# miroslavradojevic/pnr

Hardware: AMD Instinct MI355X
Metric: Mvox/s traced (Frangi+SMC step) on 1024^3 synthetic stack; % HBM roofline (higher is better)
Workload: dtype f32 (+f64 3x3 eigen-solver)

## Files before the change

### pnr_amd/csrc/devbuf.h

```cpp
#pragma once
#include <hip/hip_runtime.h>
#include <algorithm>
#include <atomic>
#include <cstdint>

namespace pnr {

inline std::atomic<int64_t> live_device_bytes{0}, live_pinned_bytes{0};

template <typename T, bool Pinned>
class Buf {
    T *p_ = nullptr;
    size_t n_ = 0;
    static std::atomic<int64_t> &live() { return Pinned ? live_pinned_bytes : live_device_bytes; }

public:
    Buf() = default;
    Buf(const Buf &) = delete;
    Buf &operator=(const Buf &) = delete;
    Buf(Buf &&o) noexcept { adopt(o.p_, o.n_), o.release(); }
    Buf &operator=(Buf &&o) noexcept
    {
        if (this != &o) adopt(o.p_, o.n_), o.release();
        return *this;
    }
    ~Buf() { reset(); }

    T *get() const { return p_; }
    explicit operator bool() const { return p_ != nullptr; }
    size_t count() const { return n_; }

    hipError_t alloc(size_t count)
    {
        reset();
        const size_t n = std::max<size_t>(count, 1);
        void *q = nullptr;
        const hipError_t e = Pinned ? hipHostMalloc(&q, n * sizeof(T), hipHostMallocDefault) : hipMalloc(&q, n * sizeof(T));
        if (e == hipSuccess) adopt((T *)q, n);
        return e;
    }
    hipError_t reserve(size_t count) { return p_ && n_ >= count ? hipSuccess : alloc(count); }
    void reset()
    {
        if (T *p = release()) (void)(Pinned ? hipHostFree(p) : hipFree(p));
    }
    void adopt(T *p, size_t count)
    {
        reset();
        p_ = p, n_ = p ? count : 0;
        live() += (int64_t)(n_ * sizeof(T));
    }
    T *release()
    {
        T *p = p_;
        live() -= (int64_t)(n_ * sizeof(T));
        p_ = nullptr, n_ = 0;
        return p;
    }
};

// ... 5 lines not shown
```

### pnr_amd/csrc/smc_phased.hip

```cpp
#include "ctx.h"
#include "replay.h"
#include "stream_sched.h"
#ifdef PNR_EXPERIMENT_HOOKS
#include "../../scripts/probes/experiments/ph_sample_hooks.h"
#else
#define PNR_HOOK_AFTER_FULL_ITEM(seg_lane, cnt)
#endif
#include "smc_device.h"
#include <algorithm>
#include <cstdlib>

namespace {

enum { FL_RES = 0, FL_STOP = 1, FL_T = 2, FL_IT = 3, FL_DONE = 4, FL_OX = 5, FL_OY = 6, FL_OZ = 7, FL_Y0 = 8, FL_Y1 = 9, FL_Z0 = 10, FL_Z1 = 11, FL_FAST = 12, FL_NCH = 13, FL_PAUSE = 14, FL_N = 16 };
constexpr int PH_THREADS = 1024;
constexpr int PH_CS = 54;
constexpr int PH_PITCH = 56;
constexpr int PH_PLANE = PH_CS * PH_PITCH;
static_assert((size_t)PH_CS * PH_PLANE <= 160 * 1024, "the cube must fit the LDS of a CU");

struct PhState {
    float *part;
    float *prior;
    int *idxres;
    float *corr;
    float *xcs;
    int *flags;
    float *stash;
    long long trace_floats;
    int stash_base;
    unsigned char *cubes;
    int *list;
    int *cnt;
    int *ctr;
    int *uidx;
    int *cmap;
    int cap;
    int np_pad;
    int W;
    int dedup;
};

__device__ __forceinline__ unsigned int pose_hash(float x, float y, float z, float vx, float vy, float vz)
{
    unsigned int h = 0x811c9dc5u;
    const unsigned int w[6] = {__float_as_uint(x), __float_as_uint(y), __float_as_uint(z), __float_as_uint(vx), __float_as_uint(vy), __float_as_uint(vz)};
#pragma unroll
    for (int i = 0; i < 6; i++) {
        h = (h ^ w[i]) * 0x9e3779b1u;
        h ^= h >> 15;
    }
    h *= 0x85ebca6bu;
    h ^= h >> 13;
    return h;
}

__device__ __forceinline__ int last_group_stride(int rem) { return rem > 32 ? 64 : (rem > 16 ? 32 : 16); }


struct CubeRows { int ox, oy, oz, y0, y1, z0, z1; };
template <class DST>
__device__ __forceinline__ void stage_cube_rows(const Vol &V, const CubeRows &R, int wv, int nwv, int lane, DST *cube32)
{
    static_assert(PH_PITCH % 4 == 0 && PH_PITCH >= PH_CS && PH_PITCH <= 64, "one dword per lane, 16 lanes per row");
// ... 535 lines not shown
        const unsigned long long sst2 = __builtin_amdgcn_s_memtime();
        atomicAdd(&g_ph_stamps[5], sst1 - sst0);
        atomicAdd(&g_ph_stamps[6], sst2 - sst1);
        atomicAdd(&g_ph_stamps[7], 1ull);
    }
#endif
}

__device__ __forceinline__ float lds_seq_sum(const float *a, int n)
{
    float s = 0.f;
    int k = 0;
    for (; k + 8 <= n; k += 8) {
        float t[8];
#pragma unroll
        for (int j = 0; j < 8; j++) t[j] = a[k + j];
#pragma unroll
        for (int j = 0; j < 8; j++) s += t[j];
    }
    for (; k < n; k++) s += a[k];
    return s;
}

__global__ __launch_bounds__(256) void ph_update(Vol V, Tab T, PhState P, int np, int np_pad, int ni, int it_arg, int lp, float Kc, float znccth,
                                                  float neff_ratio, const unsigned char *__restrict__ den, int nodepervol, TraceOut O)
{
    extern __shared__ float lds[];
    const int tid = threadIdx.x, B = blockDim.x, S = T.nsig;
    PU_STAMP(ut0);
    if ((int)blockIdx.x >= P.cnt[lp]) return;
    const int tr = P.list[lp * P.cap + blockIdx.x];
    int *fl = P.flags + (i64)tr * FL_N;
    if (fl[FL_PAUSE]) return;
    const int it = it_arg >= 0 ? it_arg : fl[FL_IT];
    float *cur = lds;
    float *prvw = cur + np * PSTRIDE;
    float *prior = prvw + np;
    float *lhood = prior + np;
    float *csw = lhood + np;
    float *corr_ks = csw + np;
    float *sneff = corr_ks + S * np_pad;
    int *sres = (int *)(sneff + 2);
    float *sxc = (float *)(sres + 2);
    const bool tail = (it == ni) || (fl[FL_STOP] != 0);
    const int pending = it - 1;
    const int resampled_prev = fl[FL_RES];
    float *gpart = P.part + (i64)tr * 2 * np * PSTRIDE;
    float *gcur = gpart + (it & 1) * np * PSTRIDE;
    const float *gprv = gpart + ((it & 1) ^ 1) * np * PSTRIDE;
    float *xc_cur = P.xcs + (i64)tr * 16 + (it & 1) * 8;
    const float *xc_pen = P.xcs + (i64)tr * 16 + ((it & 1) ^ 1) * 8;
    int *gidx = P.idxres + (i64)tr * np;
    for (int e = tid; e < S * np_pad; e += B) corr_ks[e] = P.corr[(i64)tr * S * np_pad + e];
    const int cen = fl[FL_NCH] - 1;
    const int *cmap = P.cmap + (i64)tr * P.np_pad;
    if (!tail) {
// ... 2 lines not shown
    }
    __syncthreads();
    PU_STAMP(ut1);

    if (pending >= 0 && tid == 0) {
        float best = -FLT_MAX, bs = xc_pen[6];
        for (int s = 0; s < S; s++) {
            const float cv = corr_ks[s * np_pad + cen];
            if (cv > best) { best = cv; bs = T.sig[s]; }
        }
        float *xo = O.xc + ((i64)tr * ni + pending) * 8;
        xo[0] = xc_pen[0]; xo[1] = xc_pen[1]; xo[2] = xc_pen[2]; xo[3] = xc_pen[3]; xo[4] = xc_pen[4]; xo[5] = xc_pen[5];
        xo[6] = bs; xo[7] = best;
        if ((fl[FL_STOP] == 0 || fl[FL_STOP] == 3) && best < znccth) { fl[FL_STOP] = 2; fl[FL_T] = pending; }
    }
    if (tid == 0) sres[1] = fl[FL_STOP];
    __syncthreads();
    if (tail || sres[1] != 0) {
        if (tid == 0) {
            O.T[tr] = fl[FL_T];
            O.stop[tr] = fl[FL_STOP];
            fl[FL_DONE] = 1;
        }
        return;
    }

    PU_STAMP(ut2);
    for (int k = tid; k < np; k += B) {
        float best = -FLT_MAX, bs = 0.f;
        const int ck = cmap[k];
        for (int s = 0; s < S; s++) {
            const float cv = corr_ks[s * np_pad + ck];
            if (cv > best) { best = cv; bs = T.sig[s]; }
        }
        cur[k * PSTRIDE + PCORR] = best;
        cur[k * PSTRIDE + PSIG] = bs;
        lhood[k] = expf_libm(Kc * best);
    }
    __syncthreads();

    PU_STAMP(ut3);
    const bool carry = (it > 0) && !resampled_prev;
    const int lane = tid & 63, wv = tid >> 6;
    {
        const float wnorm_prior = lds_seq_sum(prior, np);
        for (int k = tid; k < np; k += B) {
            const double base = carry ? (double)prvw[k] : (1.0 / np);
// ... 95 lines not shown
                if (ui > csw[mid]) lo = mid + 1; else hi = mid;
            }
            gidx[k] = lo;
            if (it < O.dbg_iters && O.idxres) O.idxres[((i64)tr * O.dbg_iters + it) * np + k] = lo;
        }
    }
    if (tid == 0) {
        P.list[(lp ^ 1) * P.cap + atomicAdd(&P.cnt[lp ^ 1], 1)] = tr;
        fl[FL_IT] = it + 1;
    }
    for (int e = tid; e < np * PSTRIDE; e += B) gcur[e] = cur[e];
    if (it < O.dbg_iters && O.xfilt) {
        float *dst = O.xfilt + ((i64)tr * O.dbg_iters + it) * np * PSTRIDE;
        for (int e = tid; e < np * PSTRIDE; e += B) dst[e] = cur[e];
    }
#ifdef PNR_SMC_STAMPS
    if (tid == 0) {
        const unsigned long long ut7 = __builtin_amdgcn_s_memtime();
        atomicAdd(&g_pu_stamps[8], ut1 - ut0); atomicAdd(&g_pu_stamps[9], ut2 - ut1); atomicAdd(&g_pu_stamps[10], ut3 - ut2);
        atomicAdd(&g_pu_stamps[11], ut4 - ut3); atomicAdd(&g_pu_stamps[12], ut5 - ut4); atomicAdd(&g_pu_stamps[13], ut6 - ut5);
        atomicAdd(&g_pu_stamps[14], ut7 - ut6); atomicAdd(&g_pu_stamps[15], 1ull);
    }
#endif
}

__global__ __launch_bounds__(256) void ph_snapshot(const int4 *__restrict__ src, int4 *__restrict__ dst, int n4)
{
    const int i = blockIdx.x * 256 + threadIdx.x;
    if (i < n4) dst[i] = src[i];
}

__global__ __launch_bounds__(256) void ph_poll(PhState P, float *__restrict__ s6, int do_ctl, const int *__restrict__ pause, int np_,
                                                const int *__restrict__ resume, int nr, const int *__restrict__ new_slots,
                                                const float *__restrict__ new_s6, int m, int lp, int ni, unsigned char *__restrict__ den,
                                                const i64 *__restrict__ didx, const unsigned char *__restrict__ dval, int nt)
{
    if (blockIdx.x > 0) {
        const int i = ((int)blockIdx.x - 1) * (int)blockDim.x + (int)threadIdx.x;
        if (i < nt) den_raise(den, didx[i], dval[i]);
        return;
    }
    __shared__ int kept, cntv;
    if (threadIdx.x == 0) { cntv = P.cnt[lp]; kept = 0; }
    __syncthreads();
    int *list = P.list + (size_t)lp * P.cap, *tmp = P.list + (size_t)(lp ^ 1) * P.cap;
    if (do_ctl) {
        const int n = cntv;
        for (int j = threadIdx.x; j < np_; j += blockDim.x) P.flags[(i64)pause[j] * FL_N + FL_PAUSE] = 1;
        __syncthreads();
        if (np_ > 0) {
            for (int j = threadIdx.x; j < n; j += blockDim.x) {
                const int tr = list[j];
                if (!P.flags[(i64)tr * FL_N + FL_PAUSE]) tmp[atomicAdd(&kept, 1)] = tr;
            }
            __syncthreads();
            for (int j = threadIdx.x; j < kept; j += blockDim.x) list[j] = tmp[j];
            __syncthreads();
        } else if (threadIdx.x == 0) {
            kept = n;
        }
        __syncthreads();
        const int base = kept;
        for (int j = threadIdx.x; j < nr; j += blockDim.x) {
            P.flags[(i64)resume[j] * FL_N + FL_PAUSE] = 0;
            list[base + j] = resume[j];
        }
        __syncthreads();
        if (threadIdx.x == 0) cntv = base + nr;
        __syncthreads();
    }
    if (m > 0) {
        const int base = cntv;
        for (int j = threadIdx.x; j < m; j += blockDim.x) {
            const int slot = new_slots[j];
            for (int a = 0; a < 6; a++) s6[(i64)slot * 6 + a] = new_s6[(i64)j * 6 + a];
            int *fl = P.flags + (i64)slot * FL_N;
            for (int a = 0; a < FL_N; a++) fl[a] = 0;
            fl[FL_T] = ni;
            for (int a = 0; a < 16; a++) P.xcs[(i64)slot * 16 + a] = 0.f;
            list[base + j] = slot;
        }
        __syncthreads();
        if (threadIdx.x == 0) cntv = base + m;
        __syncthreads();
    }
    if (threadIdx.x == 0) P.cnt[lp] = cntv;
}

}

struct pnr_phased {
    static constexpr int RING = 8, MAXG = 4;
    int64_t cap_traces = 0, cap_dbg = 0;
    int64_t cap_stash = 0;
    int np = 0, np_pad = 0, S = 0, ni = 0;
    long long trace_floats = 0;
    PhState P{};
    struct {
        pnr::DevBuf<float> part, prior, corr, xcs, stash;
        pnr::DevBuf<int> idxres, list, cnt, ctr, uidx, cmap;
        pnr::DevBuf<unsigned char> cubes;
    } state;
    pnr::DevBuf<float> d_s6;
    TraceOut O{};
    TraceOutBufs out;
    pnr::PinBuf<int> h_cnt;
    hipEvent_t ev[RING] = {};
    pnr::PinBuf<pnr_xest> h_xc; pnr::PinBuf<int> h_flags, h_new; pnr::PinBuf<float> h_new_s6;
    pnr::PinBuf<int> h_ctl;
    pnr::PinBuf<long long> h_den_idx[MAXG];
    pnr::PinBuf<unsigned char> h_den_val[MAXG];
    int64_t stream_cap = 0;
    int stream_ni = 0;
    hipStream_t stg[MAXG] = {};
    hipEvent_t ev_start = nullptr;
    hipEvent_t ev_state[MAXG] = {};
    hipEvent_t ev_ctl[MAXG] = {};
};

static void phased_free(pnr_phased *h)
{
    h->state = {};
    h->d_s6.reset();
    h->out.reset();
    h->P = PhState{};
    h->O = TraceOut{};
    h->cap_traces = h->cap_dbg = 0;
    h->cap_stash = 0;
}

#ifdef PNR_SMC_STAMPS
extern "C" int pnr_debug_pu_fine(unsigned long long *out4, int reset)
{
    if (out4 && hipMemcpyFromSymbol(out4, HIP_SYMBOL(g_pu_fine), 64) != hipSuccess) return -1;
    if (reset) { unsigned long long z[8] = {}; if (hipMemcpyToSymbol(HIP_SYMBOL(g_pu_fine), z, 64) != hipSuccess) return -1; }
    return 0;
}

extern "C" int pnr_debug_pu_stamps(unsigned long long *out16, int reset)
{
    if (out16 && hipMemcpyFromSymbol(out16, HIP_SYMBOL(g_pu_stamps), 128) != hipSuccess) return -1;
    if (reset) { unsigned long long z[16] = {}; if (hipMemcpyToSymbol(HIP_SYMBOL(g_pu_stamps), z, 128) != hipSuccess) return -1; }
    return 0;
}

extern "C" int pnr_debug_ph_stamps(unsigned long long *out8, int reset)
{
    if (out8 && hipMemcpyFromSymbol(out8, HIP_SYMBOL(g_ph_stamps), 64) != hipSuccess) return -1;
    if (reset) { unsigned long long z[8] = {}; if (hipMemcpyToSymbol(HIP_SYMBOL(g_ph_stamps), z, 64) != hipSuccess) return -1; }
    return 0;
}
#endif

void pnr_phased_destroy(pnr_phased *h)
{
    if (!h) return;
    for (int r = 0; r < pnr_phased::RING; r++)
        if (h->ev[r]) (void)hipEventDestroy(h->ev[r]);
    for (int g = 1; g < pnr_phased::MAXG; g++)
        if (h->stg[g]) (void)hipStreamDestroy(h->stg[g]);
    if (h->ev_start) (void)hipEventDestroy(h->ev_start);
    for (hipEvent_t &e : h->ev_state) if (e) (void)hipEventDestroy(e);
    for (hipEvent_t &e : h->ev_ctl) if (e) (void)hipEventDestroy(e);
    delete h;
}

static bool sums_deep(const pnr_ctx *c, int active, int ngroups)
{
    if (c->opt.sums_deep >= 0) return c->opt.sums_deep != 0;
    return ngroups <= 1 || active <= c->opt.sums_deep_max;
}

static int share_scales(const pnr_ctx *c, int active)
{
    return (c->opt.share_scales && c->tab.guest_mask != 0 && active >= c->opt.share_min) ? 1 : 0;
}

static int ph_tbl(int np)
{
    int t = 64;
    while (t < 2 * np) t <<= 1;
    return t;
}

static size_t ph_predict_lds(int np, int dedup) { return dedup ? (size_t)(np * 8 + 2 * ph_tbl(np)) * 4 : (size_t)np * 8; }

// ... 17 lines not shown
{
    const dim3 grid((unsigned)(active * nsplit)), blk(PH_THREADS);
    if (P.cubes) {
        if (V.l == 1) hipLaunchKernelGGL((ph_sample<PH_CS, true, true>), grid, blk, cube_bytes, st, V, T, X, P, np, ni, it, lp, active, share);
        else hipLaunchKernelGGL((ph_sample<PH_CS, false, true>), grid, blk, cube_bytes, st, V, T, X, P, np, ni, it, lp, active, share);
    } else {
        if (V.l == 1) hipLaunchKernelGGL((ph_sample<PH_CS, true, false>), grid, blk, cube_bytes, st, V, T, X, P, np, ni, it, lp, active, share);
        else hipLaunchKernelGGL((ph_sample<PH_CS, false, false>), grid, blk, cube_bytes, st, V, T, X, P, np, ni, it, lp, active, share);
    }
}

struct PhEnv {
    Vol V; Tab T; TabX X; PhState P;
    int np, ni, S, np_pad, ng, ncu, max_split, dbg_iters;
    size_t cube_bytes, upd_lds;
    long long trace_floats;
    int64_t NT;
    pnr_phased *h;
};

struct StepTimers { bool on, chain_first, chain_rest; int weight; };

static void smc_step(pnr_ctx *c, const PhEnv &E, hipStream_t st, const PhState &P, int active, int it, int lp, int x10, int sharing,
                     const unsigned char *den, const TraceOut &O, const StepTimers &tm)
{
    const int np = E.np, ni = E.ni;
    const int nsplit = pick_nsplit(active, E.ncu, E.max_split, x10), share = share_scales(c, active);
    bool chain = tm.chain_first;
    auto tic = [&] { if (tm.on) c->tic(st, chain); chain = tm.chain_rest; };
    auto toc = [&](const char *group) { if (tm.on) c->toc(group, 1, st, tm.weight); };
    tic();
    hipLaunchKernelGGL(ph_predict, dim3(active), dim3(256), ph_predict_lds(np, P.dedup), st, E.T, E.X, P, (const float *)E.h->d_s6.get(), E.V, np, ni, it, lp, PH_CS, ph_tbl(np));
    toc("smc_predict");
    if (P.cubes) {
        tic();
        hipLaunchKernelGGL(ph_cube, dim3((unsigned)(active * PH_CUBE_SPLIT)), dim3(PH_CUBE_THREADS), 0, st, E.V, P, lp, active);
        toc("smc_cube");
    }
    tic();
    launch_sample(st, E.V, E.T, E.X, P, np, ni, it, lp, active, nsplit, E.cube_bytes, share);
    toc("smc");
    tic();
    launch_sums(st, E.T, E.X, P, np, E.np_pad, ni, it, lp, active, E.ng, sums_deep(c, active, sharing), share);
    toc("smc_sums");
    tic();
    hipLaunchKernelGGL(ph_update, dim3(active), dim3(256), E.upd_lds, st, E.V, E.T, P, np, E.np_pad, ni, it, lp, c->prm.Kc, c->prm.znccth,
                       c->prm.neff_ratio, den, c->prm.nodepervol, O);
    toc("smc_update");
}

static int ensure_stash(pnr_ctx *c, pnr_phased *h, int64_t traces, long long trace_floats)
{
    if (h->cap_stash >= traces && h->P.stash) return PNR_OK;
    PNR_HIP(hipDeviceSynchronize());
    h->cap_stash = 0;
    PNR_HIP(alloc_view(h->state.stash, h->P.stash, (size_t)traces * trace_floats));
    PNR_HIP(alloc_view(h->state.cubes, h->P.cubes, (size_t)traces * PH_CS * PH_PLANE));
    h->cap_stash = traces;
    PNR_HIP(hipMemsetAsync(h->P.stash, 0, (size_t)traces * trace_floats * 4, c->stream));
    PNR_HIP(hipStreamSynchronize(c->stream));
    return PNR_OK;
}

static int phased_env(pnr_ctx *c, int64_t want, int dbg_iters, bool xfilt, bool idxres, bool neff, PhEnv &E, int64_t stash_want = 0)
{
    int rc = make_vol(c, E.V);
    if (rc) return rc;
    make_tab(c, E.T);
    const int np = c->prm.np, ni = c->prm.ni, S = E.T.nsig;
    const int np_pad = (np + 1 + 63) / 64 * 64;
    if (dbg_iters > ni) dbg_iters = ni;
    if (dbg_iters < 0) dbg_iters = 0;
    PNR_REQUIRE(want >= 1 && want < (1LL << 30), PNR_E_ARG, "bad number of traces");
    for (int s = 0; s < S; s++)
        PNR_REQUIRE(c->tab.grid[4 * s] <= 64 && c->tab.grid[4 * s + 1] <= 64 && c->tab.grid[4 * s + 2] <= 64, PNR_E_ARG,
                    "template grid axis longer than a wavefront");
    if (!c->phased) c->phased = new pnr_phased();
    pnr_phased *h = c->phased;
    if (!h->h_cnt) {
        PNR_HIP(h->h_cnt.alloc(pnr_phased::RING));
        for (int r = 0; r < pnr_phased::RING; r++) PNR_HIP(hipEventCreateWithFlags(&h->ev[r], hipEventDisableTiming));
        for (int g = 1; g < pnr_phased::MAXG; g++) PNR_HIP(hipStreamCreateWithFlags(&h->stg[g], hipStreamNonBlocking));
        PNR_HIP(hipEventCreateWithFlags(&h->ev_start, hipEventDisableTiming));
        for (hipEvent_t &e : h->ev_state) PNR_HIP(hipEventCreateWithFlags(&e, hipEventDisableTiming));
        for (hipEvent_t &e : h->ev_ctl) PNR_HIP(hipEventCreateWithFlags(&e, hipEventDisableTiming));
    }
    const int ngf = (np + 1) / 64, rem = (np + 1) - 64 * ngf, R = rem == 0 ? 0 : (rem > 32 ? 64 : (rem > 16 ? 32 : 16)), W = 64 * ngf + R;
    const long long Mtot = E.T.Mtot, trace_floats = Mtot * W;
    size_t free_b = 0, total_b = 0;
    PNR_HIP(hipMemGetInfo(&free_b, &total_b));
    size_t budget = (size_t)std::max<int64_t>(1, c->opt.stash_mb) << 20;
    const size_t have = (size_t)h->cap_stash * (size_t)h->trace_floats * 4;
    budget = std::min(budget, (free_b + have) / 2);
    const int64_t nt_max = (int64_t)(budget / ((size_t)trace_floats * 4));
    PNR_REQUIRE(nt_max >= 1, PNR_E_HIP, "not enough device memory for one trace's sample stash (%lld B)", trace_floats * 4);
    const int64_t nwaves = (want + nt_max - 1) / nt_max;
    const int64_t NT = (want + nwaves - 1) / nwaves;
    const int64_t need_dbg = NT * dbg_iters;
    if (h->cap_traces < NT || h->np != np || h->np_pad != np_pad || h->S != S || h->ni != ni || h->trace_floats != trace_floats ||
        h->cap_dbg < need_dbg || (xfilt && dbg_iters && !h->O.xfilt) || (idxres && dbg_iters && !h->O.idxres) ||
        (neff && dbg_iters && !h->O.neff)) {
        PNR_HIP(hipDeviceSynchronize());
        phased_free(h);
        const int64_t cap = NT;
        PNR_HIP(alloc_view(h->state.part, h->P.part, (size_t)cap * 2 * np * PSTRIDE));
        PNR_HIP(alloc_view(h->state.prior, h->P.prior, (size_t)cap * np));
        PNR_HIP(alloc_view(h->state.idxres, h->P.idxres, (size_t)cap * np));
        PNR_HIP(alloc_view(h->state.corr, h->P.corr, (size_t)cap * S * np_pad));
// ... 4 lines not shown
        PNR_HIP(alloc_view(h->state.ctr, h->P.ctr, (size_t)cap));
        PNR_HIP(alloc_view(h->state.uidx, h->P.uidx, (size_t)cap * np_pad));
        PNR_HIP(alloc_view(h->state.cmap, h->P.cmap, (size_t)cap * np_pad));
        PNR_HIP(h->d_s6.alloc((size_t)cap * 6));
        PNR_HIP(alloc_view(h->out.T, h->O.T, (size_t)cap));
        PNR_HIP(alloc_view(h->out.stop, h->O.stop, (size_t)cap));
        PNR_HIP(alloc_view(h->out.xc, h->O.xc, (size_t)cap * ni * 8));
        const size_t dbg_cap = (size_t)cap * dbg_iters;
        if (dbg_iters && xfilt) PNR_HIP(alloc_view(h->out.xfilt, h->O.xfilt, dbg_cap * np * PSTRIDE));
        if (dbg_iters && idxres) PNR_HIP(alloc_view(h->out.idxres, h->O.idxres, dbg_cap * np));
        if (dbg_iters && neff) PNR_HIP(alloc_view(h->out.neff, h->O.neff, dbg_cap));
        h->cap_traces = cap; h->cap_dbg = (int64_t)dbg_cap;
        h->np = np; h->np_pad = np_pad; h->S = S; h->ni = ni; h->trace_floats = trace_floats;
        PNR_HIP(hipMemsetAsync(h->P.part, 0, (size_t)cap * 2 * np * PSTRIDE * 4, c->stream));
    }
    { const int rcs = ensure_stash(c, h, stash_want > 0 ? std::min<int64_t>(stash_want, NT) : NT, trace_floats); if (rcs) return rcs; }
    E.P = h->P;
    E.P.stash_base = 0;
    E.P.trace_floats = trace_floats;
    E.P.cap = (int)h->cap_traces;
    E.P.W = W;
    E.P.np_pad = np_pad;
    E.P.dedup = np <= 1024 ? 1 : 0;
    E.X.grid = (const Grid *)c->d_grid.get(); E.X.axes = c->d_axes.get(); E.X.axes_off = c->d_axes_off.get(); E.X.wd = c->d_wd.get();
    E.X.ext_v = c->tab.ext_v; E.X.ext_uw = c->tab.ext_uw;
    for (int s2 = 0; s2 < 8; s2++) { E.X.ext_vs[s2] = s2 < S ? c->tab.ext_vs[s2] : 0.f; E.X.ext_uws[s2] = s2 < S ? c->tab.ext_uws[s2] : 0.f; }
    E.X.stash = nullptr; E.X.slot_busy = nullptr; E.X.nslots = 0; E.X.slot_floats = 0; E.X.wave_floats = 0;
    E.X.share = c->d_share.get(); E.X.grows = c->d_grows.get(); E.X.guest_mask = c->tab.guest_mask;
    hipDeviceProp_t prop;
    PNR_HIP(hipGetDeviceProperties(&prop, c->device));
    E.ncu = prop.multiProcessorCount;
    E.np = np; E.ni = ni; E.S = S; E.np_pad = np_pad; E.ng = ngf + (rem > 0 ? 1 : 0); E.dbg_iters = dbg_iters;
    E.cube_bytes = (size_t)PH_CS * PH_PLANE;
    E.upd_lds = ((size_t)np * PSTRIDE + 4 * (size_t)np + (size_t)S * np_pad + 2 + 2 + 8) * 4;
    E.trace_floats = trace_floats;
    E.NT = NT;
    E.h = h;
    E.max_split = std::max(1, c->opt.max_split);
    PNR_REQUIRE(E.upd_lds <= 160 * 1024, PNR_E_ARG, "np=%d with %d scales needs %zu B of LDS in the update step (limit 160 KB)", np, S, E.upd_lds);
    PNR_HIP(hipFuncSetAttribute((const void *)ph_update, hipFuncAttributeMaxDynamicSharedMemorySize, (int)E.upd_lds));
    PNR_HIP(hipFuncSetAttribute((const void *)ph_sample<PH_CS, false, true>, hipFuncAttributeMaxDynamicSharedMemorySize, (int)E.cube_bytes));
    PNR_HIP(hipFuncSetAttribute((const void *)ph_sample<PH_CS, true, true>, hipFuncAttributeMaxDynamicSharedMemorySize, (int)E.cube_bytes));
    PNR_HIP(hipFuncSetAttribute((const void *)ph_sample<PH_CS, false, false>, hipFuncAttributeMaxDynamicSharedMemorySize, (int)E.cube_bytes));
    PNR_HIP(hipFuncSetAttribute((const void *)ph_sample<PH_CS, true, false>, hipFuncAttributeMaxDynamicSharedMemorySize, (int)E.cube_bytes));
    if (!c->opt.cube_copy) E.P.cubes = nullptr;
    return PNR_OK;
}

int pnr_trace_run_phased(pnr_ctx *c, const pnr_seed *seeds, int64_t n, int32_t *T_out, int32_t *stop_out, pnr_xest *xc, int dbg_iters,
                         float *xfilt, int32_t *idxres, float *neff, int use_density)
{
    if (n == 0) return PNR_OK;
    PhEnv E;
    const int64_t ntr_all = 2 * n;
    int rc = phased_env(c, ntr_all, dbg_iters, xfilt != nullptr, idxres != nullptr, neff != nullptr, E);
    if (rc) return rc;
    const PhState &P = E.P;
// ... 46 lines not shown
        }
        PNR_HIP(hipGetLastError());
        PNR_HIP(hipMemcpyAsync(T_out + t0, h->O.T, (size_t)nt * 4, hipMemcpyDeviceToHost, st));
        PNR_HIP(hipMemcpyAsync(stop_out + t0, h->O.stop, (size_t)nt * 4, hipMemcpyDeviceToHost, st));
        PNR_HIP(hipMemcpyAsync(xc + t0 * ni, h->O.xc, (size_t)nt * ni * 32, hipMemcpyDeviceToHost, st));
        if (O.xfilt) PNR_HIP(hipMemcpyAsync(xfilt + t0 * dbg_iters * np * PSTRIDE, O.xfilt, (size_t)nt * dbg_iters * np * PSTRIDE * 4, hipMemcpyDeviceToHost, st));
        if (O.idxres) PNR_HIP(hipMemcpyAsync(idxres + t0 * dbg_iters * np, O.idxres, (size_t)nt * dbg_iters * np * 4, hipMemcpyDeviceToHost, st));
        if (O.neff) PNR_HIP(hipMemcpyAsync(neff + t0 * dbg_iters, O.neff, (size_t)nt * dbg_iters * 4, hipMemcpyDeviceToHost, st));
        PNR_HIP(hipStreamSynchronize(st));
    }
    return PNR_OK;
}

namespace {

struct PhasedEngine final : pnr::StreamEngine {
    pnr_ctx *c;
    PhEnv E;
    pnr_phased *h = nullptr;
    int NT = 0;
    TraceOut O{};
    struct Grp {
        PhState P; hipStream_t st; int lp = 0;
        int *h_snap, *h_flags, *h_cnt, *h_new; float *h_new_s6;
        bool p_ctl = false; int p_np = 0, p_nr = 0, p_m = 0; size_t p_nt = 0;
        long long poll_no = 0;
        hipEvent_t ev_state = nullptr;
        int running = 0;
    };
    Grp grp[pnr_phased::MAXG];
    std::string msg;
    int ngroups = 1;
    int gcap = 0;

    explicit PhasedEngine(pnr_ctx *ctx) : c(ctx) {}
    const char *error() const override { return msg.c_str(); }
    int hip_fail(hipError_t e, const char *what)
    {
        msg = std::string(what) + " failed: " + hipGetErrorString(e);
        return PNR_E_HIP;
    }
#define PE_HIP(call) do { hipError_t e_ = (call); if (e_ != hipSuccess) return hip_fail(e_, #call); } while (0)

    int init(int64_t window)
    {
        int rc = phased_env(c, window, 0, false, false, false, E, (int64_t)ngroups * 192);
        if (rc) { msg = pnr_last_error(); return rc; }
        h = E.h;
        gcap = (int)std::max<int64_t>(1, h->cap_stash / ngroups);
        NT = (int)(E.NT - (E.NT & 1));
        if (NT < 2) { msg = "not enough device memory for two trace slots"; return PNR_E_HIP; }
        const int ni = E.ni;
        if (h->stream_cap < NT || h->stream_ni != ni) {
            PE_HIP(hipDeviceSynchronize());
            h->stream_cap = 0;
            PE_HIP(h->h_xc.alloc((size_t)NT * ni));
            constexpr int MG = pnr_phased::MAXG;
            PE_HIP(h->h_flags.alloc(((size_t)NT * FL_N + 2 * MG) * MG));
            PE_HIP(h->h_new.alloc((size_t)NT * MG));
            PE_HIP(h->h_new_s6.alloc((size_t)NT * 6 * MG));
            PE_HIP(h->h_ctl.alloc((size_t)NT * 2 * MG));
            h->stream_cap = NT;
            h->stream_ni = ni;
        }
        O = h->O;
        O.xc = (float *)h->h_xc.get();
        O.dbg_iters = 0; O.xfilt = nullptr; O.idxres = nullptr; O.neff = nullptr;
        PE_HIP(hipMemsetAsync(E.P.cnt, 0, 2 * 4 * pnr_phased::MAXG, c->stream));
        PE_HIP(hipEventRecord(h->ev_start, c->stream));
        for (int g = 1; g < pnr_phased::MAXG; g++) PE_HIP(hipStreamWaitEvent(h->stg[g], h->ev_start, 0));
        for (int g = 0; g < pnr_phased::MAXG; g++) {
            Grp &q = grp[g];
            q.P = E.P;
            q.P.stash_base = (g < ngroups ? g : 0) * gcap;
            q.P.list = E.P.list + (size_t)g * 2 * E.P.cap;
            q.P.cnt = E.P.cnt + 2 * g;
            q.st = g == 0 ? c->stream : h->stg[g];
            q.ev_state = h->ev_state[g];
            q.h_snap = h->h_flags.get() + (size_t)g * ((size_t)h->stream_cap * FL_N + 2 * pnr_phased::MAXG);
            q.h_flags = q.h_snap + 2 * pnr_phased::MAXG; q.h_cnt = q.h_snap + 2 * g;
            q.h_new = h->h_new.get() + (size_t)g * h->stream_cap;
            q.h_new_s6 = h->h_new_s6.get() + (size_t)g * h->stream_cap * 6;
        }
        return PNR_OK;
    }
    int slots() const override { return NT; }
    int max_groups() const override { return pnr_phased::MAXG; }
    int admit(int g, const int *slots, const float *s6, int m) override
    {
        Grp &q = grp[g];
        PE_HIP(hipEventSynchronize(h->ev_ctl[g]));
        std::memcpy(q.h_new, slots, (size_t)m * 4);
        std::memcpy(q.h_new_s6, s6, (size_t)m * 24);
        q.p_m = m;
        return PNR_OK;
    }
    int grow_stash(int need)
    {
        const int ncap = (int)std::min<int64_t>(E.NT, std::max(need, gcap + gcap / 2));
        if (ncap < need) { msg = "a launch holds more traces than the window has slots"; return PNR_E_STATE; }
        const int rc = ensure_stash(c, h, (int64_t)ngroups * ncap, E.trace_floats);
        if (rc) { msg = pnr_last_error(); return rc; }
        gcap = ncap;
        E.P.stash = h->P.stash;
        if (E.P.cubes) E.P.cubes = h->P.cubes;
        for (int k = 0; k < pnr_phased::MAXG; k++) { grp[k].P.stash = h->P.stash; grp[k].P.cubes = E.P.cubes; grp[k].P.stash_base = (k < ngroups ? k : 0) * gcap; }
        return PNR_OK;
    }
    int launch(int g, int active, int poll, int lag) override
    {
        if (g >= ngroups) { msg = "trace group beyond the stash regions"; return PNR_E_STATE; }
        if (active > gcap) { const int rc = grow_stash(active); if (rc) return rc; }
        { const int rc = flush(g,  true); if (rc) return rc; }
        Grp &q = grp[g];
        hipStream_t st = q.st;
        q.running = active;
        int sharing = 1;
        for (int k = 0; k < ngroups; k++) sharing += (k != g && grp[k].running > 0) ? 1 : 0;
        const int x10 = c->opt.split_x10 > 0 ? c->opt.split_x10 : (sharing > 1 ? 22 : 40);
        const int pw = std::max(1, c->opt.profile_every);
        const bool prof = (q.poll_no++ % pw) == 0;
        for (int k = 0; k < poll; k++) {
            smc_step(c, E, st, q.P, active, -1, q.lp, x10, sharing, c->d_den.get(), O, StepTimers{prof, k > 0, true, pw});
            q.lp ^= 1;
            if (k == poll - 1 - lag) {
                {
                    const int n4 = (int)(((size_t)NT * FL_N + 2 * pnr_phased::MAXG) / 4);
                    hipLaunchKernelGGL(ph_snapshot, dim3((unsigned)((n4 + 255) / 256)), dim3(256), 0, st, (const int4 *)E.P.cnt, (int4 *)q.h_snap, n4);
                }
                q.h_cnt = q.h_snap + 2 * g + q.lp;
                PE_HIP(hipEventRecord(q.ev_state, st));
            }
        }
        return PNR_OK;
    }
    void idle(int g) override { grp[g].running = 0; }
    int wait(int g, int *active) override
    {
        PE_HIP(hipEventSynchronize(grp[g].ev_state));
        PE_HIP(hipGetLastError());
        *active = grp[g].h_cnt[0];
        grp[g].running = *active;
        return PNR_OK;
    }
    bool finished(int g, int slot, int *T) const override
    {
        const int *fl = grp[g].h_flags + (size_t)slot * FL_N;
        *T = fl[FL_T];
        return fl[FL_DONE] != 0;
    }
    const pnr_xest *rows(int slot) const override { return h->h_xc.get() + (size_t)slot * E.ni; }
    int progress(int g, int slot) const override
    {
        return grp[g].h_flags[(size_t)slot * FL_N + FL_IT] - 1;
    }
    int control(int g, const int *pause, int np_, const int *resume, int nr) override
    {
        Grp &q = grp[g];
        int *hc = h->h_ctl.get() + (size_t)g * 2 * h->stream_cap;
        PE_HIP(hipEventSynchronize(h->ev_ctl[g]));
        if (np_ > 0) std::memcpy(hc, pause, (size_t)np_ * 4);
        if (nr > 0) std::memcpy(hc + h->stream_cap, resume, (size_t)nr * 4);
        q.p_ctl = true; q.p_np = np_; q.p_nr = nr;
        return PNR_OK;
    }
    int flush(int g, bool followed_by_steps = false)
    {
        Grp &q = grp[g];
        if (!q.p_ctl && q.p_m == 0 && q.p_nt == 0) return PNR_OK;
        int *hc = h->h_ctl.get() + (size_t)g * 2 * h->stream_cap;
        hipLaunchKernelGGL(ph_poll, dim3((unsigned)(1 + (q.p_nt + 255) / 256)), dim3(256), 0, q.st, q.P, h->d_s6.get(), q.p_ctl ? 1 : 0, (const int *)hc, q.p_np,
                           (const int *)(hc + h->stream_cap), q.p_nr, (const int *)q.h_new, (const float *)q.h_new_s6, q.p_m, q.lp, E.ni, c->d_den.get(),
                           (const i64 *)h->h_den_idx[g].get(), (const unsigned char *)h->h_den_val[g].get(), (int)q.p_nt);
        PE_HIP(hipGetLastError());
        if (!followed_by_steps) PE_HIP(hipEventRecord(h->ev_ctl[g], q.st));
        q.p_ctl = false; q.p_np = q.p_nr = q.p_m = 0; q.p_nt = 0;
        return PNR_OK;
    }
    int end_turn(int g) override { return flush(g); }
    int settle(int g) override
    {
        { const int rc = flush(g); if (rc) return rc; }
        PE_HIP(hipStreamSynchronize(grp[g].st));
        return PNR_OK;
    }
    int density_update(const pnr::Replayer &r, int g) override
    {
        const size_t nt = r.touched.size();
        if (nt == 0) return PNR_OK;
        Grp &q = grp[g];
        if (h->h_den_val[g].count() < nt) {
            PE_HIP(hipStreamSynchronize(q.st));
            const size_t cap = std::max<size_t>(2 * nt, 1 << 16);
            PE_HIP(h->h_den_idx[g].alloc(cap));
            PE_HIP(h->h_den_val[g].alloc(cap));
        }
        PE_HIP(hipEventSynchronize(h->ev_ctl[g]));
        for (size_t i = 0; i < nt; i++) {
            h->h_den_idx[g].get()[i] = r.touched[i];
            h->h_den_val[g].get()[i] = (unsigned char)r.den_at(r.touched[i]);
        }
        q.p_nt = nt;
        return PNR_OK;
    }
    void drain() override
    {
        if (!h) return;
        for (int g = 0; g < pnr_phased::MAXG; g++) (void)hipStreamSynchronize(g == 0 ? c->stream : h->stg[g]);
    }
#undef PE_HIP
};

}

int pnr_trace_replay_stream(pnr_ctx *c, const pnr_seed *seeds, int64_t n, pnr::Replayer &r, const pnr::ShardSpec &sh, int64_t *iters_out)
{
    if (iters_out) *iters_out = 0;
    if (n == 0 && sh.world <= 1) return PNR_OK;
    pnr::SchedOptions o;
    o.window = c->opt.window; o.look0 = c->opt.look0; o.look_pct = c->opt.look_pct; o.poll = c->opt.poll; o.groups = c->opt.groups;
// ... 25 lines not shown
```

Before: 1355.

## Replace event syncs and snapshot kernel with device-published sequence words

Removes the separate ph_snapshot kernel and the hipEvent records/synchronizes used to hand state to the host. The last ph_update block, picked by an atomic ticket, now publishes changed flag rows and counts directly into coherent pinned host memory and stores a sequence number. The host spin-waits on that word with periodic stream queries. ph_poll signals completion the same way. This cuts kernel launches and event overhead per poll, at the cost of CPU spinning, system-scope fences and more complex pending-slot bookkeeping.

```diff
diff --git a/pnr_amd/csrc/devbuf.h b/pnr_amd/csrc/devbuf.h
--- a/pnr_amd/csrc/devbuf.h
+++ b/pnr_amd/csrc/devbuf.h
@@ -30,12 +30,12 @@
     explicit operator bool() const { return p_ != nullptr; }
     size_t count() const { return n_; }
 
-    hipError_t alloc(size_t count)
+    hipError_t alloc(size_t count, unsigned host_flags = hipHostMallocDefault)
     {
         reset();
         const size_t n = std::max<size_t>(count, 1);
         void *q = nullptr;
-        const hipError_t e = Pinned ? hipHostMalloc(&q, n * sizeof(T), hipHostMallocDefault) : hipMalloc(&q, n * sizeof(T));
+        const hipError_t e = Pinned ? hipHostMalloc(&q, n * sizeof(T), host_flags) : hipMalloc(&q, n * sizeof(T));
         if (e == hipSuccess) adopt((T *)q, n);
         return e;
     }
diff --git a/pnr_amd/csrc/seq_wait.h b/pnr_amd/csrc/seq_wait.h
--- /dev/null
+++ b/pnr_amd/csrc/seq_wait.h
@@ -0,0 +1,43 @@
+#pragma once
+#include <cstdint>
+#if !defined(__x86_64__) && !defined(__i386__)
+#include <thread>
+#endif
+
+namespace pnr {
+
+struct SeqWord {
+    uint32_t *word = nullptr;
+    uint32_t last = 0;
+    void bind(uint32_t *w) { word = w; last = __atomic_load_n(w, __ATOMIC_RELAXED); }
+    uint32_t next() { return ++last; }
+    bool reached() const { return __atomic_load_n(word, __ATOMIC_ACQUIRE) == last; }
+};
+
+inline void cpu_relax()
+{
+#if defined(__x86_64__) || defined(__i386__)
+    __builtin_ia32_pause();
+#else
+    std::this_thread::yield();
+#endif
+}
+
+enum SeqWait { SEQ_OK = 0, SEQ_FAILED = 1, SEQ_LOST = 2 };
+enum StreamLook { STREAM_BUSY = 0, STREAM_IDLE = 1, STREAM_ERROR = 2 };
+
+template <class Look>
+inline SeqWait seq_wait(const uint32_t *word, uint32_t want, Look &&look, unsigned every = 2048)
+{
+    for (unsigned round = 1;; round++) {
+        if (__atomic_load_n(word, __ATOMIC_ACQUIRE) == want) return SEQ_OK;
+        if (round % every == 0) {
+            const StreamLook s = look();
+            if (s == STREAM_ERROR) return SEQ_FAILED;
+            if (s == STREAM_IDLE) return __atomic_load_n(word, __ATOMIC_ACQUIRE) == want ? SEQ_OK : SEQ_LOST;
+        }
+        cpu_relax();
+    }
+}
+
+}
diff --git a/pnr_amd/csrc/smc_phased.hip b/pnr_amd/csrc/smc_phased.hip
--- a/pnr_amd/csrc/smc_phased.hip
+++ b/pnr_amd/csrc/smc_phased.hip
@@ -1,6 +1,7 @@
 #include "ctx.h"
 #include "replay.h"
 #include "stream_sched.h"
+#include "seq_wait.h"
 #ifdef PNR_EXPERIMENT_HOOKS
 #include "../../scripts/probes/experiments/ph_sample_hooks.h"
 #else
@@ -39,7 +40,25 @@
     int np_pad;
     int W;
     int dedup;
+    int *sync;
+    int *pend;
+    int pend_cap;
 };
+enum { SY_TICKET = 0, SY_NPEND = 1, SY_POLL = 2, SY_N = 16 };
+
+struct PhPublish {
+    int *flags;
+    int *cnt;
+    unsigned *word;
+    unsigned seq;
+};
+
+__device__ __forceinline__ int4 load_flags16(const int *p, int quad)
+{
+    int4 v;
+    __builtin_memcpy(&v, (const char *)__builtin_assume_aligned(p, 16) + 16 * quad, 16);
+    return v;
+}
 
 __device__ __forceinline__ unsigned int pose_hash(float x, float y, float z, float vx, float vy, float vz)
 {
@@ -621,16 +640,16 @@
     return s;
 }
 
-__global__ __launch_bounds__(256) void ph_update(Vol V, Tab T, PhState P, int np, int np_pad, int ni, int it_arg, int lp, float Kc, float znccth,
-                                                  float neff_ratio, const unsigned char *__restrict__ den, int nodepervol, TraceOut O)
-{
-    extern __shared__ float lds[];
+enum { UPD_LEFT = 1 << 30 };
+__device__ __forceinline__ int ph_update_trace(float *lds, const Vol &V, const Tab &T, const PhState &P, int np, int np_pad, int ni, int it_arg, int lp, float Kc,
+                                               float znccth, float neff_ratio, const unsigned char *__restrict__ den, int nodepervol, const TraceOut &O)
+{
     const int tid = threadIdx.x, B = blockDim.x, S = T.nsig;
     PU_STAMP(ut0);
-    if ((int)blockIdx.x >= P.cnt[lp]) return;
+    if ((int)blockIdx.x >= P.cnt[lp]) return -1;
     const int tr = P.list[lp * P.cap + blockIdx.x];
     int *fl = P.flags + (i64)tr * FL_N;
-    if (fl[FL_PAUSE]) return;
+    if (fl[FL_PAUSE]) return tr | UPD_LEFT;
     const int it = it_arg >= 0 ? it_arg : fl[FL_IT];
     float *cur = lds;
     float *prvw = cur + np * PSTRIDE;
@@ -679,7 +698,7 @@
             O.stop[tr] = fl[FL_STOP];
             fl[FL_DONE] = 1;
         }
-        return;
+        return tr | UPD_LEFT;
     }
 
     PU_STAMP(ut2);
@@ -821,22 +840,82 @@
         atomicAdd(&g_pu_stamps[14], ut7 - ut6); atomicAdd(&g_pu_stamps[15], 1ull);
     }
 #endif
-}
-
-__global__ __launch_bounds__(256) void ph_snapshot(const int4 *__restrict__ src, int4 *__restrict__ dst, int n4)
-{
-    const int i = blockIdx.x * 256 + threadIdx.x;
-    if (i < n4) dst[i] = src[i];
+    return tr;
+}
+
+__global__ __launch_bounds__(256) void ph_update(Vol V, Tab T, PhState P, int np, int np_pad, int ni, int it_arg, int lp, float Kc, float znccth,
+                                                  float neff_ratio, const unsigned char *__restrict__ den, int nodepervol, TraceOut O, PhPublish pub)
+{
+    extern __shared__ float lds[];
+    const int r = ph_update_trace(lds, V, T, P, np, np_pad, ni, it_arg, lp, Kc, znccth, neff_ratio, den, nodepervol, O);
+    const int tid = threadIdx.x;
+    if (!pub.flags) {
+        if (P.pend && tid == 0 && r >= 0 && (r & UPD_LEFT)) {
+            const int k = atomicAdd(&P.sync[SY_NPEND], 1);
+            if (k < P.pend_cap) P.pend[k] = r & ~UPD_LEFT;
+        }
+        return;
+    }
+    int *last = (int *)lds + (np * PSTRIDE + 4 * np + T.nsig * np_pad + 2 + 2 + 8);
+    if (tid == 0) {
+        if (r >= 0) {
+            const int tr = r & ~UPD_LEFT;
+            const int *fl = P.flags + (i64)tr * FL_N;
+            int4 *dst = (int4 *)(pub.flags + (i64)tr * FL_N);
+            const int4 a = load_flags16(fl, 0), b = load_flags16(fl, 1), c = load_flags16(fl, 2), d = load_flags16(fl, 3);
+            dst[0] = a; dst[1] = b; dst[2] = c; dst[3] = d;
+        }
+        __threadfence_system();
+        asm volatile("s_waitcnt vmcnt(0)" ::: "memory");
+        const int ticket = __hip_atomic_fetch_add(&P.sync[SY_TICKET], 1, __ATOMIC_RELAXED, __HIP_MEMORY_SCOPE_AGENT);
+        const int is_last = ticket == (int)gridDim.x - 1;
+        if (is_last) {
+            __builtin_amdgcn_fence(__ATOMIC_ACQUIRE, "agent");
+            asm volatile("s_waitcnt vmcnt(0)" ::: "memory");
+        }
+        *last = is_last;
+    }
+    __syncthreads();
+    if (!*last) return;
+    const int npend = min(__hip_atomic_load(&P.sync[SY_NPEND], __ATOMIC_RELAXED, __HIP_MEMORY_SCOPE_AGENT), P.pend_cap);
+    for (int e = tid; e < 4 * npend; e += blockDim.x) {
+        const int slot = P.pend[e >> 2], quad = e & 3;
+        ((int4 *)(pub.flags + (i64)slot * FL_N))[quad] = load_flags16(P.flags + (i64)slot * FL_N, quad);
+    }
+    if (tid == 0) {
+        pub.cnt[0] = __hip_atomic_load(&P.cnt[0], __ATOMIC_RELAXED, __HIP_MEMORY_SCOPE_AGENT);
+        pub.cnt[1] = __hip_atomic_load(&P.cnt[1], __ATOMIC_RELAXED, __HIP_MEMORY_SCOPE_AGENT);
+        __hip_atomic_store(&P.sync[SY_NPEND], 0, __ATOMIC_RELAXED, __HIP_MEMORY_SCOPE_AGENT);
+        __hip_atomic_store(&P.sync[SY_TICKET], 0, __ATOMIC_RELAXED, __HIP_MEMORY_SCOPE_AGENT);
+    }
+    __threadfence_system();
+    asm volatile("s_waitcnt vmcnt(0)" ::: "memory");
+    __syncthreads();
+    if (tid == 0) __hip_atomic_store(pub.word, pub.seq, __ATOMIC_RELEASE, __HIP_MEMORY_SCOPE_SYSTEM);
+}
+
+__device__ __forceinline__ void poll_done(const PhState &P, unsigned *word, unsigned seq)
+{
+    if (!word) return;
+    __syncthreads();
+    if (threadIdx.x != 0) return;
+    __threadfence();
+    asm volatile("s_waitcnt vmcnt(0)" ::: "memory");
+    if (__hip_atomic_fetch_add(&P.sync[SY_POLL], 1, __ATOMIC_RELAXED, __HIP_MEMORY_SCOPE_AGENT) != (int)gridDim.x - 1) return;
+    __hip_atomic_store(&P.sync[SY_POLL], 0, __ATOMIC_RELAXED, __HIP_MEMORY_SCOPE_AGENT);
+    __hip_atomic_store(word, seq, __ATOMIC_RELEASE, __HIP_MEMORY_SCOPE_SYSTEM);
 }
 
 __global__ __launch_bounds__(256) void ph_poll(PhState P, float *__restrict__ s6, int do_ctl, const int *__restrict__ pause, int np_,
                                                 const int *__restrict__ resume, int nr, const int *__restrict__ new_slots,
                                                 const float *__restrict__ new_s6, int m, int lp, int ni, unsigned char *__restrict__ den,
-                                                const i64 *__restrict__ didx, const unsigned char *__restrict__ dval, int nt)
+                                                const i64 *__restrict__ didx, const unsigned char *__restrict__ dval, int nt, unsigned *done_word,
+                                                unsigned done_seq)
 {
     if (blockIdx.x > 0) {
         const int i = ((int)blockIdx.x - 1) * (int)blockDim.x + (int)threadIdx.x;
         if (i < nt) den_raise(den, didx[i], dval[i]);
+        poll_done(P, done_word, done_seq);
         return;
     }
     __shared__ int kept, cntv;
@@ -845,7 +924,11 @@
     int *list = P.list + (size_t)lp * P.cap, *tmp = P.list + (size_t)(lp ^ 1) * P.cap;
     if (do_ctl) {
         const int n = cntv;
-        for (int j = threadIdx.x; j < np_; j += blockDim.x) P.flags[(i64)pause[j] * FL_N + FL_PAUSE] = 1;
+        for (int j = threadIdx.x; j < np_; j += blockDim.x) {
+            P.flags[(i64)pause[j] * FL_N + FL_PAUSE] = 1;
+            const int k = atomicAdd(&P.sync[SY_NPEND], 1);
+            if (k < P.pend_cap) P.pend[k] = pause[j];
+        }
         __syncthreads();
         if (np_ > 0) {
             for (int j = threadIdx.x; j < n; j += blockDim.x) {
@@ -884,6 +967,7 @@
         __syncthreads();
     }
     if (threadIdx.x == 0) P.cnt[lp] = cntv;
+    poll_done(P, done_word, done_seq);
 }
 
 }
@@ -913,8 +997,9 @@
     int stream_ni = 0;
     hipStream_t stg[MAXG] = {};
     hipEvent_t ev_start = nullptr;
-    hipEvent_t ev_state[MAXG] = {};
-    hipEvent_t ev_ctl[MAXG] = {};
+    static constexpr int SEQ_STRIDE = 16;
+    pnr::PinBuf<uint32_t> h_seq;
+    pnr::DevBuf<int> d_pub;
 };
 
 static void phased_free(pnr_phased *h)
@@ -959,8 +1044,6 @@
     for (int g = 1; g < pnr_phased::MAXG; g++)
         if (h->stg[g]) (void)hipStreamDestroy(h->stg[g]);
     if (h->ev_start) (void)hipEventDestroy(h->ev_start);
-    for (hipEvent_t &e : h->ev_state) if (e) (void)hipEventDestroy(e);
-    for (hipEvent_t &e : h->ev_ctl) if (e) (void)hipEventDestroy(e);
     delete h;
 }
 
@@ -1024,7 +1107,7 @@
 struct StepTimers { bool on, chain_first, chain_rest; int weight; };
 
 static void smc_step(pnr_ctx *c, const PhEnv &E, hipStream_t st, const PhState &P, int active, int it, int lp, int x10, int sharing,
-                     const unsigned char *den, const TraceOut &O, const StepTimers &tm)
+                     const unsigned char *den, const TraceOut &O, const StepTimers &tm, const PhPublish &pub = PhPublish{})
 {
     const int np = E.np, ni = E.ni;
     const int nsplit = pick_nsplit(active, E.ncu, E.max_split, x10), share = share_scales(c, active);
@@ -1047,7 +1130,7 @@
     toc("smc_sums");
     tic();
     hipLaunchKernelGGL(ph_update, dim3(active), dim3(256), E.upd_lds, st, E.V, E.T, P, np, E.np_pad, ni, it, lp, c->prm.Kc, c->prm.znccth,
-                       c->prm.neff_ratio, den, c->prm.nodepervol, O);
+                       c->prm.neff_ratio, den, c->prm.nodepervol, O, pub);
     toc("smc_update");
 }
 
@@ -1084,8 +1167,6 @@
         for (int r = 0; r < pnr_phased::RING; r++) PNR_HIP(hipEventCreateWithFlags(&h->ev[r], hipEventDisableTiming));
         for (int g = 1; g < pnr_phased::MAXG; g++) PNR_HIP(hipStreamCreateWithFlags(&h->stg[g], hipStreamNonBlocking));
         PNR_HIP(hipEventCreateWithFlags(&h->ev_start, hipEventDisableTiming));
-        for (hipEvent_t &e : h->ev_state) PNR_HIP(hipEventCreateWithFlags(&e, hipEventDisableTiming));
-        for (hipEvent_t &e : h->ev_ctl) PNR_HIP(hipEventCreateWithFlags(&e, hipEventDisableTiming));
     }
     const int ngf = (np + 1) / 64, rem = (np + 1) - 64 * ngf, R = rem == 0 ? 0 : (rem > 32 ? 64 : (rem > 16 ? 32 : 16)), W = 64 * ngf + R;
     const long long Mtot = E.T.Mtot, trace_floats = Mtot * W;
@@ -1136,6 +1217,7 @@
     E.P.W = W;
     E.P.np_pad = np_pad;
     E.P.dedup = np <= 1024 ? 1 : 0;
+    E.P.sync = nullptr; E.P.pend = nullptr; E.P.pend_cap = 0;
     E.X.grid = (const Grid *)c->d_grid.get(); E.X.axes = c->d_axes.get(); E.X.axes_off = c->d_axes_off.get(); E.X.wd = c->d_wd.get();
     E.X.ext_v = c->tab.ext_v; E.X.ext_uw = c->tab.ext_uw;
     for (int s2 = 0; s2 < 8; s2++) { E.X.ext_vs[s2] = s2 < S ? c->tab.ext_vs[s2] : 0.f; E.X.ext_uws[s2] = s2 < S ? c->tab.ext_uws[s2] : 0.f; }
@@ -1146,7 +1228,7 @@
     E.ncu = prop.multiProcessorCount;
     E.np = np; E.ni = ni; E.S = S; E.np_pad = np_pad; E.ng = ngf + (rem > 0 ? 1 : 0); E.dbg_iters = dbg_iters;
     E.cube_bytes = (size_t)PH_CS * PH_PLANE;
-    E.upd_lds = ((size_t)np * PSTRIDE + 4 * (size_t)np + (size_t)S * np_pad + 2 + 2 + 8) * 4;
+    E.upd_lds = ((size_t)np * PSTRIDE + 4 * (size_t)np + (size_t)S * np_pad + 2 + 2 + 8 + 1) * 4;
     E.trace_floats = trace_floats;
     E.NT = NT;
     E.h = h;
@@ -1239,10 +1321,11 @@
     TraceOut O{};
     struct Grp {
         PhState P; hipStream_t st; int lp = 0;
-        int *h_snap, *h_flags, *h_cnt, *h_new; float *h_new_s6;
+        int *h_state, *h_flags, *h_cnt, *h_new; float *h_new_s6;
         bool p_ctl = false; int p_np = 0, p_nr = 0, p_m = 0; size_t p_nt = 0;
         long long poll_no = 0;
-        hipEvent_t ev_state = nullptr;
+        pnr::SeqWord seq_state;
+        pnr::SeqWord seq_ctl;
         int running = 0;
     };
     Grp grp[pnr_phased::MAXG];
@@ -1271,9 +1354,10 @@
         if (h->stream_cap < NT || h->stream_ni != ni) {
             PE_HIP(hipDeviceSynchronize());
             h->stream_cap = 0;
-            PE_HIP(h->h_xc.alloc((size_t)NT * ni));
+            PE_HIP(h->h_xc.alloc((size_t)NT * ni, hipHostMallocCoherent));
             constexpr int MG = pnr_phased::MAXG;
-            PE_HIP(h->h_flags.alloc(((size_t)NT * FL_N + 2 * MG) * MG));
+            PE_HIP(h->h_flags.alloc(((size_t)NT * FL_N + 2 * MG) * MG, hipHostMallocCoherent));
+            PE_HIP(h->d_pub.alloc((size_t)MG * (SY_N + 4 * (size_t)NT)));
             PE_HIP(h->h_new.alloc((size_t)NT * MG));
             PE_HIP(h->h_new_s6.alloc((size_t)NT * 6 * MG));
             PE_HIP(h->h_ctl.alloc((size_t)NT * 2 * MG));
@@ -1283,7 +1367,12 @@
         O = h->O;
         O.xc = (float *)h->h_xc.get();
         O.dbg_iters = 0; O.xfilt = nullptr; O.idxres = nullptr; O.neff = nullptr;
+        if (!h->h_seq) {
+            PE_HIP(h->h_seq.alloc((size_t)2 * pnr_phased::MAXG * pnr_phased::SEQ_STRIDE, hipHostMallocCoherent));
+            std::memset(h->h_seq.get(), 0, h->h_seq.count() * sizeof(uint32_t));
+        }
         PE_HIP(hipMemsetAsync(E.P.cnt, 0, 2 * 4 * pnr_phased::MAXG, c->stream));
+        PE_HIP(hipMemsetAsync(h->d_pub.get(), 0, (size_t)pnr_phased::MAXG * SY_N * 4, c->stream));
         PE_HIP(hipEventRecord(h->ev_start, c->stream));
         for (int g = 1; g < pnr_phased::MAXG; g++) PE_HIP(hipStreamWaitEvent(h->stg[g], h->ev_start, 0));
         for (int g = 0; g < pnr_phased::MAXG; g++) {
@@ -1293,9 +1382,13 @@
             q.P.list = E.P.list + (size_t)g * 2 * E.P.cap;
             q.P.cnt = E.P.cnt + 2 * g;
             q.st = g == 0 ? c->stream : h->stg[g];
-            q.ev_state = h->ev_state[g];
-            q.h_snap = h->h_flags.get() + (size_t)g * ((size_t)h->stream_cap * FL_N + 2 * pnr_phased::MAXG);
-            q.h_flags = q.h_snap + 2 * pnr_phased::MAXG; q.h_cnt = q.h_snap + 2 * g;
+            q.P.sync = h->d_pub.get() + (size_t)g * SY_N;
+            q.P.pend_cap = 4 * (int)h->stream_cap;
+            q.P.pend = h->d_pub.get() + (size_t)pnr_phased::MAXG * SY_N + (size_t)g * q.P.pend_cap;
+            q.seq_state.bind(h->h_seq.get() + (size_t)pnr_phased::SEQ_STRIDE * (2 * g));
+            q.seq_ctl.bind(h->h_seq.get() + (size_t)pnr_phased::SEQ_STRIDE * (2 * g + 1));
+            q.h_state = h->h_flags.get() + (size_t)g * ((size_t)h->stream_cap * FL_N + 2 * pnr_phased::MAXG);
+            q.h_flags = q.h_state + 2 * pnr_phased::MAXG; q.h_cnt = q.h_state;
             q.h_new = h->h_new.get() + (size_t)g * h->stream_cap;
             q.h_new_s6 = h->h_new_s6.get() + (size_t)g * h->stream_cap * 6;
         }
@@ -1306,7 +1399,7 @@
     int admit(int g, const int *slots, const float *s6, int m) override
     {
         Grp &q = grp[g];
-        PE_HIP(hipEventSynchronize(h->ev_ctl[g]));
+        { const int rc = await(q, q.seq_ctl, "ph_poll"); if (rc) return rc; }
         std::memcpy(q.h_new, slots, (size_t)m * 4);
         std::memcpy(q.h_new_s6, s6, (size_t)m * 24);
         q.p_m = m;
@@ -1338,23 +1431,32 @@
         const int pw = std::max(1, c->opt.profile_every);
         const bool prof = (q.poll_no++ % pw) == 0;
         for (int k = 0; k < poll; k++) {
-            smc_step(c, E, st, q.P, active, -1, q.lp, x10, sharing, c->d_den.get(), O, StepTimers{prof, k > 0, true, pw});
+            PhPublish pub{};
+            if (k == poll - 1 - lag) {
+                pub = PhPublish{q.h_flags, q.h_state, q.seq_state.word, q.seq_state.next()};
+                q.h_cnt = q.h_state + (q.lp ^ 1);
+            }
+            smc_step(c, E, st, q.P, active, -1, q.lp, x10, sharing, c->d_den.get(), O, StepTimers{prof, k > 0, true, pw}, pub);
             q.lp ^= 1;
-            if (k == poll - 1 - lag) {
-                {
-                    const int n4 = (int)(((size_t)NT * FL_N + 2 * pnr_phased::MAXG) / 4);
-                    hipLaunchKernelGGL(ph_snapshot, dim3((unsigned)((n4 + 255) / 256)), dim3(256), 0, st, (const int4 *)E.P.cnt, (int4 *)q.h_snap, n4);
-                }
-                q.h_cnt = q.h_snap + 2 * g + q.lp;
-                PE_HIP(hipEventRecord(q.ev_state, st));
-            }
-        }
+        }
+        PE_HIP(hipGetLastError());
         return PNR_OK;
     }
     void idle(int g) override { grp[g].running = 0; }
+    int await(Grp &q, const pnr::SeqWord &sw, const char *what)
+    {
+        hipError_t qe = hipSuccess;
+        const pnr::SeqWait w = pnr::seq_wait(sw.word, sw.last, [&] {
+            qe = hipStreamQuery(q.st);
+            return qe == hipErrorNotReady ? pnr::STREAM_BUSY : (qe == hipSuccess ? pnr::STREAM_IDLE : pnr::STREAM_ERROR);
+        });
+        if (w == pnr::SEQ_FAILED) return hip_fail(qe, what);
+        if (w == pnr::SEQ_LOST) { msg = std::string(what) + " ran without storing its sequence number"; return PNR_E_STATE; }
+        return PNR_OK;
+    }
     int wait(int g, int *active) override
     {
-        PE_HIP(hipEventSynchronize(grp[g].ev_state));
+        { const int rc = await(grp[g], grp[g].seq_state, "ph_update"); if (rc) return rc; }
         PE_HIP(hipGetLastError());
         *active = grp[g].h_cnt[0];
         grp[g].running = *active;
@@ -1375,7 +1477,7 @@
     {
         Grp &q = grp[g];
         int *hc = h->h_ctl.get() + (size_t)g * 2 * h->stream_cap;
-        PE_HIP(hipEventSynchronize(h->ev_ctl[g]));
+        { const int rc = await(q, q.seq_ctl, "ph_poll"); if (rc) return rc; }
         if (np_ > 0) std::memcpy(hc, pause, (size_t)np_ * 4);
         if (nr > 0) std::memcpy(hc + h->stream_cap, resume, (size_t)nr * 4);
         q.p_ctl = true; q.p_np = np_; q.p_nr = nr;
@@ -1386,11 +1488,12 @@
         Grp &q = grp[g];
         if (!q.p_ctl && q.p_m == 0 && q.p_nt == 0) return PNR_OK;
         int *hc = h->h_ctl.get() + (size_t)g * 2 * h->stream_cap;
+        unsigned *done_word = followed_by_steps ? nullptr : q.seq_ctl.word;
+        const unsigned done_seq = followed_by_steps ? 0u : q.seq_ctl.next();
         hipLaunchKernelGGL(ph_poll, dim3((unsigned)(1 + (q.p_nt + 255) / 256)), dim3(256), 0, q.st, q.P, h->d_s6.get(), q.p_ctl ? 1 : 0, (const int *)hc, q.p_np,
                            (const int *)(hc + h->stream_cap), q.p_nr, (const int *)q.h_new, (const float *)q.h_new_s6, q.p_m, q.lp, E.ni, c->d_den.get(),
-                           (const i64 *)h->h_den_idx[g].get(), (const unsigned char *)h->h_den_val[g].get(), (int)q.p_nt);
+                           (const i64 *)h->h_den_idx[g].get(), (const unsigned char *)h->h_den_val[g].get(), (int)q.p_nt, done_word, done_seq);
         PE_HIP(hipGetLastError());
-        if (!followed_by_steps) PE_HIP(hipEventRecord(h->ev_ctl[g], q.st));
         q.p_ctl = false; q.p_np = q.p_nr = q.p_m = 0; q.p_nt = 0;
         return PNR_OK;
     }
@@ -1412,7 +1515,7 @@
             PE_HIP(h->h_den_idx[g].alloc(cap));
             PE_HIP(h->h_den_val[g].alloc(cap));
         }
-        PE_HIP(hipEventSynchronize(h->ev_ctl[g]));
+        { const int rc = await(q, q.seq_ctl, "ph_poll"); if (rc) return rc; }
         for (size_t i = 0; i < nt; i++) {
             h->h_den_idx[g].get()[i] = r.touched[i];
             h->h_den_val[g].get()[i] = (unsigned char)r.den_at(r.touched[i]);
```

Result: no change. 1348 (-0.6%).
